# arielnetworks/tidal-wave

Hardware: AMD Instinct MI355X
Metric: image-pairs/sec @1080p Farneback (default params), 1/2/4/8 MI355X (higher is better)
Workload: dtype f32

## Files before the change

include/twflow_debug.h:

```cpp
#ifndef TWFLOW_DEBUG_H
#define TWFLOW_DEBUG_H

#include "twflow.h"

#ifdef __cplusplus
extern "C" {
#endif

int tw_debug_graphs(tw_engine* e);

tw_status tw_debug_check_size(int width, int height);

int tw_debug_occupancy(char* buf, int cap);

int tw_debug_stamps(tw_engine* e, unsigned long long* out);

int tw_debug_stamps_ex(tw_engine* e, unsigned long long* out, int n);

tw_status tw_debug_copy_rate(tw_engine* e, size_t bytes, int reps, double* gbps);

enum tw_debug_family {
    TW_DF_PYR_K3 = 0,
    TW_DF_PYR_K3F,
    TW_DF_PYR_23,
// ... 17 lines not shown
    TW_DF_SPAN_SCAN,
    TW_DF_PNG_UNFILTER,
    TW_DF_SPAN_SCAN_SEG,
    TW_DF_BLUR_SOLVE4Q,
    TW_DF_PAIR_SAME,
    TW_DF_RESIZE_U8,
    TW_DF_FLOW_INIT,
    TW_DF_FLOW_EXPORT,
    TW_DF_COUNT
};

int tw_debug_launch_counts(tw_engine* e, unsigned long long* counts, unsigned long long* last_z, int n, int reset);

int tw_debug_flow_iter_plan(const tw_engine* e, int width, int height, int npairs, int* out, int n);

int tw_debug_blur_plan(const tw_engine* e, int width, int height, int level, int npairs, int update, int quads, int* out, int n);

int tw_debug_same_flags(tw_engine* e, unsigned* out, int n);

tw_status tw_debug_png_kernel_time(tw_engine* e, const tw_png_rows* img, int waves, int iters, float* avg_us);

const char* tw_debug_family_name(int family);

int tw_debug_memory(tw_engine* e, unsigned long long* out, int n);

#ifdef __cplusplus
}
#endif
#endif
```

tidal-wave_amd/csrc/twflow.hip:

```cpp
#include "twflow_kernels.hip.h"

#include <hip/hip_runtime.h>
#include <unistd.h>

#include <dlfcn.h>
#include <float.h>
#include <math.h>
#include <stdio.h>
#include <stdlib.h>
#include <string.h>

#include <array>
#include <chrono>
#include <map>
#include <mutex>
#include <string>
#include <tuple>
#include <utility>
#include <vector>

#include "../../include/twflow.h"
#include "../../include/twflow_debug.h"

using namespace twk;
// ... 77 lines not shown
            if (sx >= sw - 1) { fx = 0; sx = sw - 1; }
        }
        t.xofs[dx] = sx;
        t.alpha[2 * dx] = 1.f - fx;
        t.alpha[2 * dx + 1] = fx;
    }
    for (int dy = 0; dy < dh; dy++) {
        float fy = (float)((dy + 0.5) * scale_y - 0.5);
        int sy = cv_floor(fy);
        fy -= sy;
        t.yofs[dy] = sy;
        t.beta[2 * dy] = 1.f - fy;
        t.beta[2 * dy + 1] = fy;
    }
}

struct AreaTab {
    int mode = 2, ix = 1, iy = 1;
    std::vector<int> xstart, xsi, ystart, ysi;
    std::vector<float> xalpha, ybeta;
};
void area_tab_1d(int ssize, int dsize, double scale, std::vector<int>& start, std::vector<int>& si, std::vector<float>& alpha)
{
    start.assign(dsize + 1, 0);
    si.clear();
    alpha.clear();
    for (int dx = 0; dx < dsize; dx++) {
        start[dx] = (int)si.size();
        const double fsx1 = dx * scale;
        const double fsx2 = fsx1 + scale;
// ... 127 lines not shown
    int w = 0, h = 0, ld = 0;
    long long ps = 0;
    double sigma = 0, scale = 1;
    int ksize = 3;
    int chunk = 1;
    int *d_xofs = nullptr, *d_yofs = nullptr;
    float *d_alpha = nullptr, *d_beta = nullptr, *d_kern = nullptr;
    int mode = 1, xmax = 0, nrows_max = 0;
    float h_kern[3] = {0, 0, 0};
    std::vector<float> h_taps;
    int pitch_b = 0;
    int gen_th = PYR_TH, gen_nrows_max = 0;
    int *d_uxofs = nullptr, *d_uyofs = nullptr;
    float *d_ualpha = nullptr, *d_ubeta = nullptr;
    int uxmax = 0;
};

struct Plan {
    int w0 = 0, h0 = 0;
    bool fused23 = false;
    float k19[24] = {0}, k9[16] = {0};
    int levels = 0;
    std::vector<LevelPlan> lv;
    int init_mode = 0, init_ix = 1, init_iy = 1, init_tw = 0;
    int *d_ixs = nullptr, *d_ixi = nullptr, *d_iys = nullptr, *d_iyi = nullptr;
    float *d_ixa = nullptr, *d_iyb = nullptr;
    std::vector<void*> owned;
    size_t owned_bytes = 0;
    unsigned long long last_use = 0;
};
// ... 504 lines not shown
            (s = upload_vec(e, pl, t.alpha, &L.d_alpha)) || (s = upload_vec(e, pl, t.beta, &L.d_beta)) ||
            (s = upload_vec(e, pl, kern, &L.d_kern))) {
            free_plan(pl);
            return s;
        }
        if (k < pl->levels) {
            const LevelPlan& P = pl->lv[k + 1];
            ResizeTab u;
            make_resize_tab(P.w, P.h, L.w, L.h, u);
            if (u.mode == 2) {
                e->err = "unexpected area-fast flow resize";
                free_plan(pl);
                return TW_E_UNSUPPORTED;
            }
            L.uxmax = u.xmax;
            if ((s = upload_vec(e, pl, u.xofs, &L.d_uxofs)) || (s = upload_vec(e, pl, u.yofs, &L.d_uyofs)) ||
                (s = upload_vec(e, pl, u.alpha, &L.d_ualpha)) || (s = upload_vec(e, pl, u.beta, &L.d_ubeta))) {
                free_plan(pl);
                return s;
            }
        }
    }
    {
        const LevelPlan& C = pl->lv[pl->levels];
        AreaTab t;
        make_area_tab(w0, h0, C.w, C.h, t);
        pl->init_mode = t.mode;
        pl->init_ix = t.ix;
        pl->init_iy = t.iy;
        if (t.mode == 1) {
// ... 406 lines not shown
    return e->p.pyrIterations > 0 && e->scan_fused && span == 10 && e->win_m == 15 && !e->box;
}
int balanced_launch_pairs(int n, int chunk)
{
    const int nlaunch = (n + chunk - 1) / chunk;
    return nlaunch > 0 ? (n + nlaunch - 1) / nlaunch : 1;
}
struct FlowUps {
    const float* prev;
    int pw, ph, pld;
    long long pfps;
    const int *xofs, *yofs;
    const float *alpha, *beta;
    int xmax;
    float scale;
};
template <typename A>
void set_upsample(A& a, const FlowUps& u)
{
    a.prev = u.prev;
    a.pw = u.pw;
    a.ph = u.ph;
    a.pld = u.pld;
    a.pfps = u.pfps;
    a.xofs = u.xofs;
    a.alpha = u.alpha;
    a.yofs = u.yofs;
    a.beta = u.beta;
    a.xmax = u.xmax;
    a.scale = u.scale;
// ... 28 lines not shown
        if (sg > 1 && nt < e->fi_minsteps) break;
        const long long wgs = (long long)nstrips * sg * npairs;
        const long long rounds = (wgs + slots - 1) / slots;
        const double cost = (double)rounds * (nt + 7 * 0.25);
        if (cost < best_cost) {
            best_cost = cost;
            best_seg = sg;
        }
    }
    FlowIterPlan fp;
    fp.strips = nstrips;
    fp.nt = (nsteps + best_seg - 1) / best_seg;
    fp.segments = (nsteps + fp.nt - 1) / fp.nt;
    fp.nt_last = nsteps - (fp.segments - 1) * fp.nt;
    return fp;
}
void launch_flow_iter(tw_engine* e, hipStream_t st, int w, int h, int ld, long long ps, const float* R, const float* flow_in,
                      long long fps_in, float* flow_out, long long fps_out, const FlowUps* ups, int npairs, int level,
                      const unsigned* same = nullptr)
{
    FlowIterArgs a;
    memset(&a, 0, sizeof(a));
    a.same = same;
    a.R = R;
    a.flow_in = flow_in;
    a.flow_out = flow_out;
    a.w = w;
    a.h = h;
    a.ld = ld;
    a.ps = ps;
// ... 6 lines not shown
    a.dbg = (unsigned long long*)e->dbg_stamps;
#endif
    const FlowIterPlan fp = flow_iter_plan(e, w, h, npairs);
    a.nt = fp.nt;
    const dim3 grid(fp.strips, fp.segments, npairs);
    ProfScope pscope(e, st, TW_K_BLUR_SOLVE, level);
    if (ups) set_upsample(a, *ups);
#ifdef TW_VARIANTS
    if (e->fi_nt == 512) {
        if (ups) TW_LAUNCH(e, TW_DF_FLOW_ITER_UPS, (tw_flow_iter<15, 1, 512>), grid, dim3(512), 0, st, a);
        else if (a.zero_flow) TW_LAUNCH(e, TW_DF_FLOW_ITER_ZERO, (tw_flow_iter<15, 2, 512>), grid, dim3(512), 0, st, a);
        else TW_LAUNCH(e, TW_DF_FLOW_ITER, (tw_flow_iter<15, 0, 512>), grid, dim3(512), 0, st, a);
        return;
    }
#endif
    if (ups) {
        TW_LAUNCH(e, TW_DF_FLOW_ITER_UPS, (tw_flow_iter<15, 1>), grid, dim3(1024), 0, st, a);
    } else if (a.zero_flow) {
        TW_LAUNCH(e, TW_DF_FLOW_ITER_ZERO, (tw_flow_iter<15, 2>), grid, dim3(1024), 0, st, a);
    } else {
        TW_LAUNCH(e, TW_DF_FLOW_ITER, (tw_flow_iter<15, 0>), grid, dim3(1024), 0, st, a);
    }
}

#ifndef TW_4Y_ILP
#define TW_4Y_ILP 2, 2, 2
#endif
struct BlurKernel {
    void (*kern)(BlurArgs);
    int family;
    int block;
// ... 175 lines not shown
    } else {
        void (*const kern)(BlurArgs) = c.k->kern;
        TW_LAUNCH(e, c.k->family, kern, c.grid, dim3(c.k->block), c.lds, st, a);
    }
}

void launch_update(tw_engine* e, hipStream_t st, const Plan* pl, int k, const float* R, float* flow,
                   const float* prev, float* M, int npairs, const SideJob* side = nullptr, bool* side_used = nullptr,
                   bool init_flow = false)
{
    const LevelPlan& L = pl->lv[k];
    const bool up = k < pl->levels;
    FlowUps ups;
    if (up) {
        const LevelPlan& P = pl->lv[k + 1];
        ups = FlowUps{prev, P.w, P.h, P.ld, P.ps, L.d_uxofs, L.d_uyofs, L.d_ualpha, L.d_ubeta, L.uxmax, (float)(1. / e->p.pyrScale)};
    }
    UpdArgs a = upd_args(R, flow, M, L.w, L.h, L.ld, L.ps, up ? &ups : nullptr);
    a.store_flow = e->p.pyrIterations == 0 ? 1 : 0;
    ProfScope pscope(e, st, TW_K_UPDATE_MATRICES, k);
    if (up) {
        launch_upd_kernel<true>(e, st, L.w, L.h, npairs, a, side, side_used);
    } else {
        a.zero_flow = init_flow ? 0 : 1;
        launch_upd_kernel<false>(e, st, L.w, L.h, npairs, a, side, side_used);
    }
}

void launch_area_init(tw_engine* e, hipStream_t st, const Plan* pl, float* flow, int j0, int nc)
{
    const LevelPlan& L = pl->lv[pl->levels];
// ... 695 lines not shown
        side_next++;
    }


    void enqueue_flow_iter_chain(const LevelChunk& ch)
    {
        const int k = ch.k, nc = ch.nc;
        const LevelPlan& L = pl->lv[k];
        const int nfi = ch.grid_only ? it - 1 : it;
        float* buf[2] = {ch.flow_cur, ch.M0};
        if (ch.init_lv) launch_area_init(e, ch.ls, pl, buf[nfi & 1], ch.j0, nc);
        FlowUps ups;
        if (k < pl->levels) {
            const LevelPlan& Pv = pl->lv[k + 1];
            ups = FlowUps{ch.flow_prev, Pv.w, Pv.h, Pv.ld, Pv.ps, L.d_uxofs, L.d_uyofs, L.d_ualpha, L.d_ubeta, L.uxmax,
                          (float)(1. / e->p.pyrScale)};
        }
        for (int i = 0; i < nfi; i++) {
            float* out = buf[(nfi - 1 - i) & 1];
            const float* in = i == 0 ? (ch.init_lv ? buf[nfi & 1] : nullptr) : buf[(nfi - i) & 1];
            launch_flow_iter(e, ch.ls, L.w, L.h, L.ld, L.ps, ch.R, in, L.ps, out, L.ps,
                             (i == 0 && k < pl->levels) ? &ups : nullptr, nc, k, same_flags_of(ch));
        }
        if (!ch.grid_only) return;
        UpdArgs u;
        memset(&u, 0, sizeof(u));
        u.R = ch.R;
        u.flow = ch.flow_cur;
        u.M = ch.M1;
        u.w = L.w;
        u.h = L.h;
// ... 1473 lines not shown
    const char* why = "";
    return size_status(width, height, &why);
}

extern "C" int tw_debug_flow_iter_plan(const tw_engine* e, int width, int height, int npairs, int* out, int n)
{
    if (!e) return -1;
    if (!out || width < 1 || height < 1 || npairs < 1) return 0;
    const FlowIterPlan fp = flow_iter_plan(e, width, height, npairs);
    const int v[4] = {fp.strips, fp.segments, fp.nt, fp.nt_last};
    int i = 0;
    for (; i < n && i < 4; i++) out[i] = v[i];
    return i;
}

extern "C" int tw_debug_blur_plan(const tw_engine* e, int width, int height, int level, int npairs, int update, int quads, int* out, int n)
{
    if (!e) return -1;
    if (!out || width < 1 || height < 1 || npairs < 1) return 0;
    const BlurChoice c = choose_blur(e, width, height, npairs, level, update != 0, quads != 0);
    const int v[9] = {c.k->family, c.k->block, c.k->tw, c.k->th, c.xsh, (int)c.grid.x, (int)c.grid.y, c.small, c.forced ? 1 : 0};
    int i = 0;
    for (; i < n && i < 9; i++) out[i] = v[i];
    return i;
}

extern "C" int tw_debug_launch_counts(tw_engine* e, unsigned long long* counts, unsigned long long* last_z, int n, int reset)
{
    if (!e) return -1;
    for (int i = 0; i < n && i < TW_DF_COUNT; i++) {
// ... 218 lines not shown
        switch (kclass) {
            case TW_K_PYR:
                e->img_aligned4 = (npx0 % 4 == 0) ? 1 : 0;
                launch_pyr(e, st, pl, level, tab, width, I, 2 * npairs);
                break;
            case TW_K_POLYEXP: return launch_polyexp(e, st, L.w, L.h, L.ld, L.ps, I, R, 2 * npairs, level);
            case TW_K_UPDATE_MATRICES: launch_update(e, st, pl, level, R, fl, pf, M0, npairs); break;
            case TW_K_BLUR_SOLVE:
                if (flags & 12) {
                    if (!flow_iter_eligible(e, L.w, L.h)) return TW_E_UNSUPPORTED;
                    FlowUps ups;
                    const bool up = (flags & 8) && level < pl->levels;
                    if (up) {
                        const LevelPlan& Pv = pl->lv[level + 1];
                        ups = FlowUps{pf, Pv.w, Pv.h, Pv.ld, Pv.ps, L.d_uxofs, L.d_uyofs, L.d_ualpha, L.d_ubeta, L.uxmax,
                                      (float)(1. / e->p.pyrScale)};
                    }
                    launch_flow_iter(e, st, L.w, L.h, L.ld, L.ps, R, up ? nullptr : fl, L.ps, M1, L.ps, up ? &ups : nullptr,
                                     npairs, level);
                    break;
                }
                launch_blur(e, st, BlurLaunch{L.w, L.h, L.ld, L.ps, (i & 1) ? M1 : M0, (i & 1) ? M0 : M1, fl, R, (flags & 2) ? 0 : 1,
                                              level, npairs});
                break;
            case TW_K_SCAN: {
                GatherArgs g;
                g.flow = fl; g.fzs = 2 * L.ps; g.fps = L.ps; g.ld = L.ld; g.span = span;
                g.gw = (L.w + span - 1) / span; g.gh = (L.h + span - 1) / span; g.g = grid;
                TW_LAUNCH(e, TW_DF_SPAN_GATHER, tw_span_gather, dim3((g.gw + 63) / 64, (g.gh + 3) / 4, npairs), dim3(256), 0, st, g);
                ScanArgs a;
                a.g = grid; a.span = span; a.gw = g.gw; a.gh = g.gh; a.thr2 = 4.0; a.count = cnt;
// ... 51 lines not shown
{
    ResizeTab u;
    make_resize_tab(pw, ph, w, h, u);
    if (u.mode == 2) return TW_E_UNSUPPORTED;
    const int pld = round_up(pw, 32);
    const long long pps = (long long)pld * ph;
    float* d_p = t.alloc<float>(pps * 2);
    int *d_xo = t.alloc<int>(w), *d_yo = t.alloc<int>(h);
    float *d_al = t.alloc<float>(2 * (size_t)w), *d_be = t.alloc<float>(2 * (size_t)h);
    if (!d_p || !d_xo || !d_yo || !d_al || !d_be) return TW_E_NOMEM;
    TW_TRY(up_planes(e, d_p, pld, pps, prev2, pw, ph, 2));
    TW_TRY(h2d_sync(e, d_xo, u.xofs.data(), (size_t)w * 4));
    TW_TRY(h2d_sync(e, d_yo, u.yofs.data(), (size_t)h * 4));
    TW_TRY(h2d_sync(e, d_al, u.alpha.data(), (size_t)w * 8));
    TW_TRY(h2d_sync(e, d_be, u.beta.data(), (size_t)h * 8));
    *ups = FlowUps{d_p, pw, ph, pld, pps, d_xo, d_yo, d_al, d_be, u.xmax, (float)(1. / e->p.pyrScale)};
    return TW_OK;
}
}

extern "C" {

tw_status tw_stage_pyr_level(tw_engine* e, const uint8_t* img, int w0, int h0, int level, float* I, int* w, int* h)
{
    if (!e || !img || !I) return TW_E_BAD_PARAMETER;
    tw_status r = check_dims(e, w0, h0);
    if (r) return r;
    TW_HIP(e, hipSetDevice(e->device));
    Plan* pl = nullptr;
    if ((r = get_plan(e, w0, h0, &pl))) return r;
    if (level < 0 || level > pl->levels) return TW_E_BAD_PARAMETER;
// ... 319 lines not shown
```

tidal-wave_amd/csrc/twflow_kernels.hip.h:

```cpp
#pragma once
#include <hip/hip_runtime.h>
#include <stdint.h>
#include <type_traits>

namespace twk {

typedef float __attribute__((ext_vector_type(4))) f32x4;
typedef const float __attribute__((address_space(1))) * gptr_cf;
typedef const char __attribute__((address_space(1))) * gptr_cc;

__device__ __forceinline__ gptr_cf sgpr_base(const float* p)
{
    gptr_cf g = (gptr_cf)p;
    asm volatile("" : "+s"(g));
    return g;
}
__device__ __forceinline__ float gload(gptr_cf row, unsigned byte_off)
{
    return *(gptr_cf)((gptr_cc)row + byte_off);
}
typedef float __attribute__((address_space(1))) * gptr_f;
typedef char __attribute__((address_space(1))) * gptr_c;
__device__ __forceinline__ gptr_f sgpr_base_w(float* p)
{
// ... 1859 lines not shown
                    }
                }
            }
        }
    }
}
template <int MH, int COLS, int HALO, int TH, bool FUSED, int VILP = 2, int HILP = 2, int SUNROLL = 2, bool QPRE = true, bool VPRE = true>
__global__ __launch_bounds__(COLS) __attribute__((amdgpu_waves_per_eu(4, 8))) void tw_blur_solve4(BlurArgs a)
{
    __shared__ __attribute__((aligned(16))) float sm[5][TH][COLS];
    tw_blur_solve4_body<MH, COLS, HALO, TH, FUSED, VILP, HILP, SUNROLL, QPRE, VPRE>(a, hw_grid(), hw_block(), sm);
}

constexpr int FI_TH = 5, FI_SC = 190, FI_PITCH = 192;
constexpr int FI_SC_512 = 94, FI_PITCH_512 = 96;
struct FlowIterArgs {
    const float* R;
    const float* flow_in;
    float* flow_out;
    int w, h, ld;
    long long ps, fps_in, fps_out;
    int nt;
    int zero_flow;
    const float* prev;
    int pw, ph, pld;
    long long pfps;
    const int* xofs;
    const float* alpha;
    const int* yofs;
    const float* beta;
// ... 9 lines not shown
#define TW_FI_SKIP(bit) (a.dbg_skip & (bit))
#define TW_FI_SYNC() do { if (!TW_FI_SKIP(16)) __syncthreads(); } while (0)
#define TW_FI_STAMP(i)                                                                                                   \
    do {                                                                                                                 \
        if (a.dbg && (tid == 0 || tid == NT / 2 + 64) && fi_blin < 32 && st >= 40 && st < 48)                              \
            a.dbg[(((size_t)fi_blin * 2 + (tid ? 1 : 0)) * 8 + (st - 40)) * 8 + (i)] = __builtin_amdgcn_s_memtime();       \
    } while (0)
#else
#define TW_FI_SKIP(bit) false
#define TW_FI_SYNC() __syncthreads()
#define TW_FI_STAMP(i) do { } while (0)
#endif
template <int MH, int MODE, int NT = 1024>
__global__ __launch_bounds__(NT) __attribute__((amdgpu_waves_per_eu(4, 4))) void tw_flow_iter(FlowIterArgs a)
{
    constexpr bool UPS = MODE == 1;
#ifndef TW_FI_DEEP
#define TW_FI_DEEP 1
#endif
    constexpr bool DEEP = TW_FI_DEEP && MODE != 1 && NT == 1024;
#ifndef TW_FI_DIST
#define TW_FI_DIST 0
#endif
#define TW_FI_P(ph, sl) ((ph) * 8 + (sl))
    constexpr int DIST[4][10] = {
        {TW_FI_P(0, 0), TW_FI_P(0, 0), TW_FI_P(1, 0), TW_FI_P(1, 0), TW_FI_P(1, 1), TW_FI_P(1, 1), TW_FI_P(2, 0), TW_FI_P(2, 0), TW_FI_P(2, 0), TW_FI_P(2, 0)},
        {TW_FI_P(0, 1), TW_FI_P(0, 3), TW_FI_P(1, 0), TW_FI_P(1, 1), TW_FI_P(1, 2), TW_FI_P(1, 3), TW_FI_P(2, 0), TW_FI_P(2, 0), TW_FI_P(2, 1), TW_FI_P(2, 1)},
        {TW_FI_P(2, 0), TW_FI_P(2, 0), TW_FI_P(2, 0), TW_FI_P(2, 0), TW_FI_P(2, 0), TW_FI_P(2, 0), TW_FI_P(2, 0), TW_FI_P(2, 0), TW_FI_P(2, 0), TW_FI_P(2, 0)},
        {TW_FI_P(0, 0), TW_FI_P(0, 0), TW_FI_P(0, 1), TW_FI_P(0, 1), TW_FI_P(0, 2), TW_FI_P(0, 2), TW_FI_P(0, 3), TW_FI_P(0, 3), TW_FI_P(0, 4), TW_FI_P(0, 4)},
    };
#ifndef TW_FI_UDIST
#define TW_FI_UDIST 1
#endif
    constexpr int UDIST[2][15] = {
        {TW_FI_P(0, 0), TW_FI_P(0, 0), TW_FI_P(0, 1), TW_FI_P(0, 1), TW_FI_P(0, 2), TW_FI_P(0, 2), TW_FI_P(1, 0), TW_FI_P(1, 0), TW_FI_P(1, 1), TW_FI_P(1, 1),
         TW_FI_P(0, 0), TW_FI_P(0, 1), TW_FI_P(0, 2), TW_FI_P(0, 3), TW_FI_P(0, 4)},
        {TW_FI_P(0, 0), TW_FI_P(0, 0), TW_FI_P(0, 1), TW_FI_P(0, 2), TW_FI_P(0, 3), TW_FI_P(0, 4), TW_FI_P(1, 0), TW_FI_P(1, 1), TW_FI_P(1, 2), TW_FI_P(1, 3),
         TW_FI_P(2, 1), TW_FI_P(2, 1), TW_FI_P(2, 1), TW_FI_P(2, 1), TW_FI_P(2, 1)},
    };
    constexpr int TH = FI_TH, SC = NT == 1024 ? FI_SC : FI_SC_512, P = NT == 1024 ? FI_PITCH : FI_PITCH_512, OUT = SC - 2 * MH,
                  RING = TH + 2 * MH, NCH = RING / TH, NB = NCH + 1;
    static_assert(RING % TH == 0 && SC <= P && TH * SC <= NT && TH == 5 && OUT % 4 == 0 && 5 * TH * (OUT / 4) <= NT && (NB & (NB - 1)) == 0, "geometry");
    constexpr int VWAVES = (TH * SC + 63) / 64;
    constexpr bool SPLIT = VWAVES * 64 < NT;
    __shared__ __attribute__((aligned(16))) float blk[NB][5][TH][P];
    const int tid = threadIdx.x;
    int bx, seg, z;
    xcd_remap(bx, seg, z);
    const unsigned fi_blin = blockIdx.x + gridDim.x * (blockIdx.y + gridDim.y * blockIdx.z);
    (void)fi_blin;
    const WinCoef& c = a.c;
    const float* __restrict__ R0 = a.R + (long long)(2 * z) * 5 * a.ps;
    const float* __restrict__ R1 = R0 + ((a.same && a.same[z]) ? 0 : 5 * a.ps);
    const float* __restrict__ fin = a.flow_in + (long long)z * 2 * a.fps_in;
    float* __restrict__ fout = a.flow_out + (long long)z * 2 * a.fps_out;
    const bool cth = tid < TH * SC;
    const int cr = cth ? tid / SC : 0, cc = cth ? tid - cr * SC : 0;
    const int xc = clampi(bx * OUT - MH + cc, 0, a.w - 1);
    const int ys = seg * a.nt * TH;
    const int nsteps = min(a.nt, (a.h - ys + TH - 1) / TH);
// ... 42 lines not shown
            f.p[1] = bload(rsp, b0 + sx1b, 0u);
            f.p[2] = bload(rsp, b1 + sxb, 0u);
            f.p[3] = bload(rsp, b1 + sx1b, 0u);
            f.p[4] = bload(rsp, b0 + sxb, prev_p1);
            f.p[5] = bload(rsp, b0 + sx1b, prev_p1);
            f.p[6] = bload(rsp, b1 + sxb, prev_p1);
            f.p[7] = bload(rsp, b1 + sx1b, prev_p1);
        } else if constexpr (MODE == 2) {
            f.p[0] = f.p[1] = 0.f;
        } else {
            const unsigned o = (unsigned)(yc * a.ld + xc) * 4u;
            f.p[0] = bload(rsf, o, 0u);
            f.p[1] = bload(rsf, o, fin_p1);
        }
    };
    auto flow_value = [&](const FlowIn& f, float& dx, float& dy) {
        if constexpr (UPS) {
            const float t0x = two ? f.p[0] * ua0 + f.p[1] * ua1 : f.p[0] * 1.f;
            const float t1x = two ? f.p[2] * ua0 + f.p[3] * ua1 : f.p[2] * 1.f;
            const float t0y = two ? f.p[4] * ua0 + f.p[5] * ua1 : f.p[4] * 1.f;
            const float t1y = two ? f.p[6] * ua0 + f.p[7] * ua1 : f.p[6] * 1.f;
            dx = (t0x * f.b0 + t1x * f.b1) * a.scale + 0.f;
            dy = (t0y * f.b0 + t1y * f.b1) * a.scale + 0.f;
        } else {
            asm volatile("v_mov_b32 %0, %2\n\tv_mov_b32 %1, %3" : "=&v"(dx), "=&v"(dy) : "v"(f.p[0]), "v"(f.p[1]));
        }
    };
    gptr_cf r0b[5], r1b[5];
#pragma unroll
    for (int ch = 0; ch < 5; ch++) {
        r0b[ch] = sgpr_base(R0 + ch * a.ps);
        r1b[ch] = sgpr_base(R1 + ch * a.ps);
    }
    unsigned go0 = 0, go1 = 0;
    unsigned gq = 0;
    auto gather_r0 = [&](int ch, float q[5]) { q[ch] = gload(r0b[ch], gq); };
    auto gather_head = [&](int k, float dx, float dy, float q[5], UpdTaps& T, bool with_r0) {
        const int yc = row_of(k);
        gq = (unsigned)(yc * a.ld + xc) * 4u;
        if (with_r0) {
// ... 50 lines not shown
        ytab_issue(0);
        flow_issue(0, fcur);
        ytab_issue(1);
#pragma unroll 1
        for (int k = 0; k < NCH; k++) {
            flow_issue(k + 1, fnext);
            ytab_issue(k + 2);
            flow_value(fcur, dx, dy);
            gather_issue(k, dx, dy, q, T);
            combine_store(k, dx, dy, q, T);
            fcur = fnext;
        }
        if constexpr (DEEP) {
            FlowIn f2;
            flow_issue(NCH + 1, f2);
            ytab_issue(NCH + 2);
            flow_value(fnext, dx, dy);
            gather_head(NCH, dx, dy, q, T, false);
#pragma unroll
            for (int ch = 0; ch < 5; ch++) gather_plane(ch, T);
            flow_value(f2, dxb, dyb);
            gather_head(NCH + 1, dxb, dyb, q, Tb, false);
        } else {
        flow_value(fnext, dx, dy);
        gather_head(NCH, dx, dy, q, T, true);
        }
    }
    __syncthreads();

    constexpr int NQ = OUT / 4;
    const bool hth = tid < 5 * TH * NQ;
// ... 57 lines not shown
                    for (int u = 0; u < 15; u++)
                        if (UDIST[TW_FI_UDIST][u] == TW_FI_P(1, j)) {
                            if (u < 10) gather_half(u >> 1, u & 1, Tl);
                            else gather_r0(u - 10, ql);
                        }
                } else {
                    if (j < 2) gather_plane(HPLANE0 + j, Tl);
                }
            }
            __builtin_amdgcn_sched_barrier(0);
        }
        *(f32x4*)&blk[s0][hp][hr][4 * hq] = o;
    };

    if (SPLIT && tid >= VWAVES * 64) {
#pragma unroll 1
        for (int st = 0; st < nsteps; st++) {
            const int s0 = st & (NB - 1), bX = (st + NCH) & (NB - 1);
            TW_FI_SYNC();
            if (hth && !TW_FI_SKIP(4)) h_phase(s0, bX, std::false_type(), T, q);
            TW_FI_SYNC();
            s_phase(st, s0);
            TW_FI_SYNC();
        }
        return;
    }

    auto step = [&](int st, float (&qc)[5], float (&qn)[5]) {
        const bool more = st + 1 < nsteps;
        const int s0 = st & (NB - 1), bX = (st + NCH) & (NB - 1);
        TW_FI_STAMP(0);
        if (cth) {
            flow_issue(st + NCH + 1, fnext);
            ytab_issue(st + NCH + 2);
            gq = (unsigned)(row_of(st + NCH + 1) * a.ld + xc) * 4u;
            __builtin_amdgcn_sched_barrier(0);
            float wv[RING];
#pragma unroll
            for (int j = 0; j < NCH; j++) {
                const float* bj = &blk[(s0 + j) & (NB - 1)][cr][0][cc];
#pragma unroll
                for (int r = 0; r < TH; r++) wv[TH * j + r] = bj[r * P];
            }
            float* vout = &blk[bX][cr][0][cc];
#pragma unroll
            for (int r = 0; r < TH; r++) {
                float sv = wv[r + MH] * c.k[0];
#pragma unroll
                for (int i = 1; i <= MH; i++) sv += (wv[r + MH + i] + wv[r + MH - i]) * c.k[i];
// ... 23 lines not shown
        TW_FI_STAMP(4);

        s_phase(st, s0);
        __builtin_amdgcn_sched_barrier(0);
        TW_FI_STAMP(5);
        if (cth) {
            if (more && !TW_FI_SKIP(1)) combine_store(st + NCH, dx, dy, qc, T);
            __builtin_amdgcn_sched_barrier(0);
            if constexpr (UPS) {
#pragma unroll
                for (int u = 10; u < 15; u++)
                    if (UDIST[TW_FI_UDIST][u] == TW_FI_P(2, 1)) gather_r0(u - 10, qn);
                __builtin_amdgcn_sched_barrier(0);
            }
            TW_FI_STAMP(6);
            flow_value(fnext, dx, dy);
            gather_head(st + NCH + 1, dx, dy, qn, T, false);
            __builtin_amdgcn_sched_barrier(0);
        }
        TW_FI_STAMP(7);
        TW_FI_SYNC();
    };
    auto step_deep = [&](int st, float& dxc, float& dyc, UpdTaps& Tc, float& dxn, float& dyn, UpdTaps& Tn) {
        const bool more = st + 1 < nsteps;
        const int s0 = st & (NB - 1), bX = (st + NCH) & (NB - 1);
        TW_FI_STAMP(0);
        if (cth) {
            flow_issue(st + NCH + 2, fnext);
            ytab_issue(st + NCH + 3);
            gq = (unsigned)(row_of(st + NCH) * a.ld + xc) * 4u;
            __builtin_amdgcn_sched_barrier(0);
            float wv[RING];
#pragma unroll
            for (int j = 0; j < NCH; j++) {
                const float* bj = &blk[(s0 + j) & (NB - 1)][cr][0][cc];
#pragma unroll
                for (int r = 0; r < TH; r++) wv[TH * j + r] = bj[r * P];
            }
            float* vout = &blk[bX][cr][0][cc];
#pragma unroll
            for (int r = 0; r < TH; r++) {
                float sv = wv[r + MH] * c.k[0];
#pragma unroll
                for (int i = 1; i <= MH; i++) sv += (wv[r + MH + i] + wv[r + MH - i]) * c.k[i];
// ... 16 lines not shown
        s_phase(st, s0);
        __builtin_amdgcn_sched_barrier(0);
        TW_FI_STAMP(5);
        if (cth) {
#pragma unroll
            for (int u = 0; u < 10; u++)
                if (DIST[TW_FI_DIST][u] == TW_FI_P(2, 0)) gather_half(u >> 1, u & 1, Tn);
            __builtin_amdgcn_sched_barrier(0);
            if (more && !TW_FI_SKIP(1)) combine_store(st + NCH, dxc, dyc, q, Tc);
            __builtin_amdgcn_sched_barrier(0);
#pragma unroll
            for (int u = 0; u < 10; u++)
                if (DIST[TW_FI_DIST][u] == TW_FI_P(2, 1)) gather_half(u >> 1, u & 1, Tn);
            __builtin_amdgcn_sched_barrier(0);
            TW_FI_STAMP(6);
            flow_value(fnext, dxc, dyc);
            gather_head(st + NCH + 2, dxc, dyc, q, Tc, false);
            __builtin_amdgcn_sched_barrier(0);
        }
        TW_FI_STAMP(7);
        TW_FI_SYNC();
    };
    if constexpr (DEEP) {
        int st = 0;
#pragma unroll 1
        for (; st + 1 < nsteps; st += 2) {
            step_deep(st, dx, dy, T, dxb, dyb, Tb);
            step_deep(st + 1, dxb, dyb, Tb, dx, dy, T);
        }
        if (st < nsteps) step_deep(st, dx, dy, T, dxb, dyb, Tb);
        return;
// ... 1913 lines not shown
```

tidal-wave_amd/twflow.py:

```python
import collections
import ctypes as C
import os

import numpy as np

_HERE = os.path.dirname(os.path.abspath(__file__))
LIB_PATH = os.path.join(_HERE, "libtwflow.so")

TW_OK, TW_E_BAD_PARAMETER, TW_E_BAD_IMAGE_FORMAT, TW_E_DONT_MATCH_SIZE = 0, 1, 2, 3
TW_E_DEVICE, TW_E_NOMEM, TW_E_UNSUPPORTED, TW_E_BUSY = 4, 5, 6, 7
K_PYR, K_POLYEXP, K_UPDATE_MATRICES, K_BLUR_SOLVE, K_SCAN = 0, 1, 2, 3, 4
KERNEL_NAMES = {K_PYR: "tw_pyr_level", K_POLYEXP: "tw_polyexp", K_UPDATE_MATRICES: "tw_update_matrices",
                K_BLUR_SOLVE: "tw_blur_solve", K_SCAN: "tw_span_scan"}


class Params(C.Structure):
    _fields_ = [("pyrScale", C.c_double), ("pyrLevels", C.c_int), ("winSize", C.c_int),
                ("pyrIterations", C.c_int), ("polyN", C.c_int), ("polySigma", C.c_double),
                ("flags", C.c_int)]


class Vector(C.Structure):
    _fields_ = [("x", C.c_int), ("y", C.c_int), ("dx", C.c_double), ("dy", C.c_double)]

# ... 21 lines not shown
OPT_POLYEXP_F32 = 2

SYMBOLS = [
    "tw_default_params", "tw_abi_version", "tw_has_variants", "tw_device_count", "tw_device_pci_bus_id", "tw_engine_create", "tw_engine_destroy", "tw_strerror",
    "tw_last_error", "tw_flow_u8", "tw_diff_u8", "tw_submit_u8", "tw_submit_png8", "tw_submit_dev", "tw_flush", "tw_wait",
    "tw_submit_u8_flow", "tw_submit_png8_flow", "tw_submit_dev_flow",
    "tw_submit_u8_flow_init", "tw_submit_png8_flow_init", "tw_submit_dev_flow_init",
    "tw_submit_u8_sized", "tw_submit_png8_sized", "tw_submit_dev_sized", "tw_stage_resize_u8",
    "tw_png_on_device", "tw_submit_png", "tw_stage_png_decode",
    "tw_grid_capacity", "tw_dev_alloc", "tw_dev_free", "tw_dev_upload", "tw_dev_download", "tw_host_alloc", "tw_host_free", "tw_host_register", "tw_host_unregister", "tw_set_option",
    "tw_prof_select", "tw_prof_read",
    "tw_algorithmic_bytes", "tw_algorithmic_bytes_launch", "tw_level_runs_flow_iter", "tw_algorithmic_bytes_pair", "tw_min_traffic_bytes_pair", "tw_num_levels", "tw_level_chunk", "tw_bench_stage", "tw_stage_pyr_level", "tw_stage_pyr_fused23", "tw_stage_pyr_fused01",
    "tw_stage_png_unfilter", "tw_stage_polyexp", "tw_stage_update_matrices", "tw_stage_flow_upsample_update", "tw_stage_blur_solve", "tw_stage_flow_iter",
    "tw_debug_graphs", "tw_debug_occupancy", "tw_debug_stamps", "tw_debug_stamps_ex", "tw_debug_copy_rate",
    "tw_debug_launch_counts", "tw_debug_family_name", "tw_debug_memory", "tw_debug_check_size", "tw_debug_flow_iter_plan",
    "tw_debug_blur_plan", "tw_debug_same_flags", "tw_debug_png_kernel_time",
]


PNG_PLAIN_GRAY = -1


class PngRows(C.Structure):
    _fields_ = [("rows", C.POINTER(C.c_uint8)), ("width", C.c_int), ("height", C.c_int), ("color_type", C.c_int),
                ("bit_depth", C.c_int), ("palette", C.POINTER(C.c_uint8)), ("palette_entries", C.c_int)]

    def __init__(self, rows, width, height, color_type=PNG_PLAIN_GRAY, bit_depth=8, palette=None, palette_entries=None):
        super().__init__()
        self._rows = np.ascontiguousarray(rows, np.uint8)
        self._palette = None if palette is None else np.ascontiguousarray(palette, np.uint8)
# ... 128 lines not shown
    L.tw_algorithmic_bytes_launch.argtypes = [vp, C.c_int, C.c_int, C.c_int, C.c_int, C.c_int]
    L.tw_algorithmic_bytes_launch.restype = C.c_double
    L.tw_level_runs_flow_iter.argtypes = [vp, C.c_int, C.c_int, C.c_int, C.c_int]
    L.tw_level_runs_flow_iter.restype = C.c_int
    u64p = C.POINTER(C.c_uint64)
    L.tw_debug_launch_counts.argtypes = [vp, u64p, u64p, C.c_int, C.c_int]
    L.tw_debug_launch_counts.restype = C.c_int
    L.tw_debug_family_name.argtypes = [C.c_int]
    L.tw_debug_family_name.restype = C.c_char_p
    L.tw_debug_memory.argtypes = [vp, u64p, C.c_int]
    L.tw_debug_memory.restype = C.c_int
    L.tw_debug_check_size.argtypes = [C.c_int, C.c_int]
    L.tw_debug_check_size.restype = C.c_int
    L.tw_debug_flow_iter_plan.argtypes = [vp, C.c_int, C.c_int, C.c_int, ip, C.c_int]
    L.tw_debug_flow_iter_plan.restype = C.c_int
    L.tw_debug_blur_plan.argtypes = [vp, C.c_int, C.c_int, C.c_int, C.c_int, C.c_int, C.c_int, ip, C.c_int]
    L.tw_debug_blur_plan.restype = C.c_int
    L.tw_debug_same_flags.argtypes = [vp, C.POINTER(C.c_uint), C.c_int]
    L.tw_debug_same_flags.restype = C.c_int
    return L


FlowIterPlan = collections.namedtuple("FlowIterPlan", "strips segments nt nt_last")
BlurPlan = collections.namedtuple("BlurPlan", "family block tile_cols rows xsh grid_x grid_y small forced")


class LaunchCounts(dict):

    def flow_iter(self):
        return self["tw_flow_iter"] + self["tw_flow_iter_ups"] + self["tw_flow_iter_zero"]


def abi_version():
    return lib().tw_abi_version()


def default_params(**kw):
    p = Params()
# ... 363 lines not shown
    def algorithmic_bytes(self, kclass, level, w, h, npairs=None):
        if npairs is None:
            return self._L.tw_algorithmic_bytes(self._h, kclass, level, w, h)
        return self._L.tw_algorithmic_bytes_launch(self._h, kclass, level, w, h, npairs)

    def level_runs_flow_iter(self, w, h, level, npairs):
        return self._L.tw_level_runs_flow_iter(self._h, w, h, level, npairs) == 1

    def flow_iter_plan(self, w, h, npairs=1):
        v = (C.c_int * 4)()
        n = self._L.tw_debug_flow_iter_plan(self._h, w, h, npairs, v, 4)
        if n != 4:
            raise TwError(TW_E_BAD_PARAMETER, "tw_debug_flow_iter_plan(%d, %d, %d) returned %d" % (w, h, npairs, n))
        return FlowIterPlan(*v)

    def blur_plan(self, w, h, level=-1, npairs=1, update=False, quads=False):
        v = (C.c_int * 9)()
        n = self._L.tw_debug_blur_plan(self._h, w, h, level, npairs, int(bool(update)), int(bool(quads)), v, 9)
        if n != 9:
            raise TwError(TW_E_BAD_PARAMETER, "tw_debug_blur_plan(%d, %d, %d, %d) returned %d" % (w, h, level, npairs, n))
        return BlurPlan(self._L.tw_debug_family_name(v[0]).decode(), *v[1:8], bool(v[8]))

    def same_flags(self):
        v = (C.c_uint * self.slots)()
        n = self._L.tw_debug_same_flags(self._h, v, self.slots)
        if n < 0:
            raise TwError(TW_E_DEVICE, "tw_debug_same_flags returned %d" % n)
        return [int(v[i]) for i in range(n)]

    def launch_counts(self, reset=False):
# ... 100 lines not shown
```

Baseline: 4983.

## Stage upsampled previous-level flow in LDS via idle wave in flow_iter

Adds a staged variant of the upsampling flow-iteration kernel in which the spare wave beyond the compute waves prefetches the previous-level flow rows and row interpolation weights into a shared-memory staging array one step ahead. Compute threads then read the bilinear taps from LDS instead of issuing per-thread global gathers and y-table loads on the critical path. The plan decides per level whether the source column span fits the staging width, and otherwise falls back to the old path. This costs extra LDS and adds a producer pipeline that could affect occupancy or synchronization.

Measured after the change: 5007 (median of 6 runs). No clear change (+0.5%).

```diff
diff --git a/include/twflow_debug.h b/include/twflow_debug.h
--- a/include/twflow_debug.h
+++ b/include/twflow_debug.h
@@ -55,6 +55,8 @@
 
 int tw_debug_flow_iter_plan(const tw_engine* e, int width, int height, int npairs, int* out, int n);
 
+int tw_debug_flow_iter_ups_plan(const tw_engine* e, int prev_width, int prev_height, int width, int height, int* out, int n);
+
 int tw_debug_blur_plan(const tw_engine* e, int width, int height, int level, int npairs, int update, int quads, int* out, int n);
 
 int tw_debug_same_flags(tw_engine* e, unsigned* out, int n);
diff --git a/tidal-wave_amd/csrc/twflow.hip b/tidal-wave_amd/csrc/twflow.hip
--- a/tidal-wave_amd/csrc/twflow.hip
+++ b/tidal-wave_amd/csrc/twflow.hip
@@ -115,6 +115,12 @@
         t.beta[2 * dy + 1] = fy;
     }
 }
+
+struct FlowIterStage {
+    int rows, cols, bytes;
+    bool staged;
+};
+FlowIterStage flow_iter_ups_stage(const std::vector<int>& xofs, int w);
 
 struct AreaTab {
     int mode = 2, ix = 1, iy = 1;
@@ -272,6 +278,7 @@
     int *d_uxofs = nullptr, *d_uyofs = nullptr;
     float *d_ualpha = nullptr, *d_ubeta = nullptr;
     int uxmax = 0;
+    bool ustaged = false;
 };
 
 struct Plan {
@@ -806,6 +813,7 @@
                 return TW_E_UNSUPPORTED;
             }
             L.uxmax = u.xmax;
+            L.ustaged = flow_iter_ups_stage(u.xofs, L.w).staged;
             if ((s = upload_vec(e, pl, u.xofs, &L.d_uxofs)) || (s = upload_vec(e, pl, u.yofs, &L.d_uyofs)) ||
                 (s = upload_vec(e, pl, u.alpha, &L.d_ualpha)) || (s = upload_vec(e, pl, u.beta, &L.d_ubeta))) {
                 free_plan(pl);
@@ -1242,6 +1250,7 @@
     const float *alpha, *beta;
     int xmax;
     float scale;
+    bool staged;
 };
 template <typename A>
 void set_upsample(A& a, const FlowUps& u)
@@ -1300,6 +1309,21 @@
     fp.segments = (nsteps + fp.nt - 1) / fp.nt;
     fp.nt_last = nsteps - (fp.segments - 1) * fp.nt;
     return fp;
+}
+FlowIterStage flow_iter_ups_stage(const std::vector<int>& xofs, int w)
+{
+    const int OUT = FI_SC - 30;
+    int cols = 0;
+    for (int bx = 0; bx * OUT < w; bx++) {
+        const int xl = std::min(std::max(bx * OUT - 15, 0), w - 1), xr = std::min(bx * OUT - 15 + FI_SC - 1, w - 1);
+        cols = std::max(cols, xofs[xr] - xofs[xl] + 2);
+    }
+    FlowIterStage s;
+    s.rows = 2 * FI_TH;
+    s.cols = cols;
+    s.bytes = (2 * s.rows * cols + 2 * FI_TH + 2 * FI_PITCH) * 4;
+    s.staged = cols <= FI_STG_COLS;
+    return s;
 }
 void launch_flow_iter(tw_engine* e, hipStream_t st, int w, int h, int ld, long long ps, const float* R, const float* flow_in,
                       long long fps_in, float* flow_out, long long fps_out, const FlowUps* ups, int npairs, int level,
@@ -1336,7 +1360,9 @@
         return;
     }
 #endif
-    if (ups) {
+    if (ups && ups->staged) {
+        TW_LAUNCH(e, TW_DF_FLOW_ITER_UPS, (tw_flow_iter<15, 3>), grid, dim3(1024), 0, st, a);
+    } else if (ups) {
         TW_LAUNCH(e, TW_DF_FLOW_ITER_UPS, (tw_flow_iter<15, 1>), grid, dim3(1024), 0, st, a);
     } else if (a.zero_flow) {
         TW_LAUNCH(e, TW_DF_FLOW_ITER_ZERO, (tw_flow_iter<15, 2>), grid, dim3(1024), 0, st, a);
@@ -1542,7 +1568,7 @@
     FlowUps ups;
     if (up) {
         const LevelPlan& P = pl->lv[k + 1];
-        ups = FlowUps{prev, P.w, P.h, P.ld, P.ps, L.d_uxofs, L.d_uyofs, L.d_ualpha, L.d_ubeta, L.uxmax, (float)(1. / e->p.pyrScale)};
+        ups = FlowUps{prev, P.w, P.h, P.ld, P.ps, L.d_uxofs, L.d_uyofs, L.d_ualpha, L.d_ubeta, L.uxmax, (float)(1. / e->p.pyrScale), L.ustaged};
     }
     UpdArgs a = upd_args(R, flow, M, L.w, L.h, L.ld, L.ps, up ? &ups : nullptr);
     a.store_flow = e->p.pyrIterations == 0 ? 1 : 0;
@@ -2268,7 +2294,7 @@
         if (k < pl->levels) {
             const LevelPlan& Pv = pl->lv[k + 1];
             ups = FlowUps{ch.flow_prev, Pv.w, Pv.h, Pv.ld, Pv.ps, L.d_uxofs, L.d_uyofs, L.d_ualpha, L.d_ubeta, L.uxmax,
-                          (float)(1. / e->p.pyrScale)};
+                          (float)(1. / e->p.pyrScale), L.ustaged};
         }
         for (int i = 0; i < nfi; i++) {
             float* out = buf[(nfi - 1 - i) & 1];
@@ -3772,6 +3798,20 @@
     return i;
 }
 
+extern "C" int tw_debug_flow_iter_ups_plan(const tw_engine* e, int prev_width, int prev_height, int width, int height, int* out, int n)
+{
+    if (!e) return -1;
+    if (!out || prev_width < 1 || prev_height < 1 || width < 1 || height < 1) return 0;
+    ResizeTab u;
+    make_resize_tab(prev_width, prev_height, width, height, u);
+    if (u.mode == 2) return 0;
+    const FlowIterStage s = flow_iter_ups_stage(u.xofs, width);
+    const int v[5] = {s.staged && e->fi_nt != 512 ? 1 : 0, s.rows, s.cols, s.bytes, FI_STG_DWORDS * 4};
+    int i = 0;
+    for (; i < n && i < 5; i++) out[i] = v[i];
+    return i;
+}
+
 extern "C" int tw_debug_blur_plan(const tw_engine* e, int width, int height, int level, int npairs, int update, int quads, int* out, int n)
 {
     if (!e) return -1;
@@ -4020,7 +4060,7 @@
                     if (up) {
                         const LevelPlan& Pv = pl->lv[level + 1];
                         ups = FlowUps{pf, Pv.w, Pv.h, Pv.ld, Pv.ps, L.d_uxofs, L.d_uyofs, L.d_ualpha, L.d_ubeta, L.uxmax,
-                                      (float)(1. / e->p.pyrScale)};
+                                      (float)(1. / e->p.pyrScale), L.ustaged};
                     }
                     launch_flow_iter(e, st, L.w, L.h, L.ld, L.ps, R, up ? nullptr : fl, L.ps, M1, L.ps, up ? &ups : nullptr,
                                      npairs, level);
@@ -4102,7 +4142,7 @@
     TW_TRY(h2d_sync(e, d_yo, u.yofs.data(), (size_t)h * 4));
     TW_TRY(h2d_sync(e, d_al, u.alpha.data(), (size_t)w * 8));
     TW_TRY(h2d_sync(e, d_be, u.beta.data(), (size_t)h * 8));
-    *ups = FlowUps{d_p, pw, ph, pld, pps, d_xo, d_yo, d_al, d_be, u.xmax, (float)(1. / e->p.pyrScale)};
+    *ups = FlowUps{d_p, pw, ph, pld, pps, d_xo, d_yo, d_al, d_be, u.xmax, (float)(1. / e->p.pyrScale), flow_iter_ups_stage(u.xofs, w).staged};
     return TW_OK;
 }
 }
diff --git a/tidal-wave_amd/csrc/twflow_kernels.hip.h b/tidal-wave_amd/csrc/twflow_kernels.hip.h
--- a/tidal-wave_amd/csrc/twflow_kernels.hip.h
+++ b/tidal-wave_amd/csrc/twflow_kernels.hip.h
@@ -1897,6 +1897,10 @@
 
 constexpr int FI_TH = 5, FI_SC = 190, FI_PITCH = 192;
 constexpr int FI_SC_512 = 94, FI_PITCH_512 = 96;
+constexpr int FI_STG_COLS = 98, FI_STG_LINES = 4 * FI_TH;
+constexpr int FI_STG_ROWTAB = FI_STG_LINES * FI_STG_COLS, FI_STG_COLTAB = FI_STG_ROWTAB + 2 * FI_TH;
+constexpr int FI_STG_DWORDS = FI_STG_COLTAB + 2 * FI_PITCH;
+constexpr int FI_LDS_BYTES = 163840;
 struct FlowIterArgs {
     const float* R;
     const float* flow_in;
@@ -1936,11 +1940,16 @@
 template <int MH, int MODE, int NT = 1024>
 __global__ __launch_bounds__(NT) __attribute__((amdgpu_waves_per_eu(4, 4))) void tw_flow_iter(FlowIterArgs a)
 {
-    constexpr bool UPS = MODE == 1;
+    constexpr bool STG = MODE == 3;
+    constexpr bool UPS = MODE == 1 || STG;
+    static_assert(!STG || NT == 1024, "the staged upsample needs wave 15");
 #ifndef TW_FI_DEEP
 #define TW_FI_DEEP 1
 #endif
-    constexpr bool DEEP = TW_FI_DEEP && MODE != 1 && NT == 1024;
+#ifndef TW_FI_STG_DEEP
+#define TW_FI_STG_DEEP 1
+#endif
+    constexpr bool DEEP = TW_FI_DEEP && MODE != 1 && (!STG || TW_FI_STG_DEEP) && NT == 1024;
 #ifndef TW_FI_DIST
 #define TW_FI_DIST 0
 #endif
@@ -1966,6 +1975,10 @@
     constexpr int VWAVES = (TH * SC + 63) / 64;
     constexpr bool SPLIT = VWAVES * 64 < NT;
     __shared__ __attribute__((aligned(16))) float blk[NB][5][TH][P];
+    __shared__ __attribute__((aligned(16))) float stg[STG ? FI_STG_DWORDS : 1];
+    static_assert(!STG || sizeof(blk) + FI_STG_DWORDS * 4 <= FI_LDS_BYTES, "staging array");
+    constexpr int CP = FI_STG_COLS;
+    constexpr int KOFF = NCH + (DEEP ? 2 : 1);
     const int tid = threadIdx.x;
     int bx, seg, z;
     xcd_remap(bx, seg, z);
@@ -2038,7 +2051,7 @@
             f.p[1] = bload(rsf, o, fin_p1);
         }
     };
-    auto flow_value = [&](const FlowIn& f, float& dx, float& dy) {
+    auto ups_value = [&](const FlowIn& f, bool two, float ua0, float ua1, float& dx, float& dy) {
         if constexpr (UPS) {
             const float t0x = two ? f.p[0] * ua0 + f.p[1] * ua1 : f.p[0] * 1.f;
             const float t1x = two ? f.p[2] * ua0 + f.p[3] * ua1 : f.p[2] * 1.f;
@@ -2046,8 +2059,80 @@
             const float t1y = two ? f.p[6] * ua0 + f.p[7] * ua1 : f.p[6] * 1.f;
             dx = (t0x * f.b0 + t1x * f.b1) * a.scale + 0.f;
             dy = (t0y * f.b0 + t1y * f.b1) * a.scale + 0.f;
+        }
+    };
+    auto flow_value = [&](const FlowIn& f, float& dx, float& dy) {
+        if constexpr (UPS) {
+            ups_value(f, two, ua0, ua1, dx, dy);
         } else {
             asm volatile("v_mov_b32 %0, %2\n\tv_mov_b32 %1, %3" : "=&v"(dx), "=&v"(dy) : "v"(f.p[0]), "v"(f.p[1]));
+        }
+    };
+    const int xlo = STG ? clampi(bx * OUT - MH, 0, a.w - 1) : 0;
+    int sxbase = 0;
+    unsigned stg_tap = 0;
+    if constexpr (STG) {
+        sxbase = a.xofs[xlo];
+        stg_tap = (unsigned)(2 * cr * CP + sx - sxbase) | (two ? 0u : 0x80000000u);
+        if (tid < SC) {
+            float* ct = &stg[FI_STG_COLTAB + xc - xlo];
+            ct[0] = ua0;
+            ct[P] = ua1;
+        }
+    }
+    auto flow_staged = [&](float& dx, float& dy) {
+        if constexpr (STG) {
+            const float* ct = &stg[FI_STG_COLTAB + xc - xlo];
+            const float* sp = &stg[stg_tap & 0x7FFFFFFFu];
+            FlowIn f;
+#pragma unroll
+            for (int pl = 0; pl < 2; pl++) {
+                f.p[4 * pl] = sp[pl * 2 * TH * CP];
+                f.p[4 * pl + 1] = sp[pl * 2 * TH * CP + 1];
+                f.p[4 * pl + 2] = sp[pl * 2 * TH * CP + CP];
+                f.p[4 * pl + 3] = sp[pl * 2 * TH * CP + CP + 1];
+            }
+            f.b0 = stg[FI_STG_ROWTAB + 2 * cr];
+            f.b1 = stg[FI_STG_ROWTAB + 2 * cr + 1];
+            ups_value(f, !(stg_tap >> 31), ct[0], ct[P], dx, dy);
+        }
+    };
+    const int wl = tid & 63;
+    const unsigned svo0 = STG ? (unsigned)min(sxbase + wl, a.pw - 1) * 4u : 0u, svo1 = STG ? (unsigned)min(sxbase + wl + 64, a.pw - 1) * 4u : 0u;
+    float sreg[STG ? 2 * FI_STG_LINES : 1];
+    float sb0 = 0.f, sb1 = 0.f;
+    int ssy = 0;
+    auto stg_row = [&](int k) { return clampi(ys - MH + TH * k + min(wl, TH - 1), 0, a.h - 1); };
+    auto stg_ytab = [&](int k) { ssy = a.yofs[stg_row(k)]; };
+    auto stg_issue = [&](int k) {
+        const int yc = stg_row(k);
+        sb0 = a.beta[2 * yc];
+        sb1 = a.beta[2 * yc + 1];
+#pragma unroll
+        for (int r = 0; r < TH; r++) {
+            const int sy = __builtin_amdgcn_readlane(ssy, r);
+#pragma unroll
+            for (int hf = 0; hf < 2; hf++) {
+                const unsigned so = (unsigned)(clampi(sy + hf, 0, a.ph - 1) * a.pld) * 4u;
+#pragma unroll
+                for (int pl = 0; pl < 2; pl++) {
+                    const int line = pl * 2 * TH + 2 * r + hf;
+                    sreg[2 * line] = bload(rsp, svo0, so + (pl ? prev_p1 : 0u));
+                    sreg[2 * line + 1] = bload(rsp, svo1, so + (pl ? prev_p1 : 0u));
+                }
+            }
+        }
+    };
+    auto stg_write = [&]() {
+#pragma unroll
+        for (int line = 0; line < FI_STG_LINES; line++) stg[line * CP + wl] = sreg[2 * line];
+        if (wl + 64 < CP) {
+#pragma unroll
+            for (int line = 0; line < FI_STG_LINES; line++) stg[line * CP + wl + 64] = sreg[2 * line + 1];
+        }
+        if (wl < TH) {
+            stg[FI_STG_ROWTAB + 2 * wl] = sb0;
+            stg[FI_STG_ROWTAB + 2 * wl + 1] = sb1;
         }
     };
     gptr_cf r0b[5], r1b[5];
@@ -2128,7 +2213,7 @@
         if constexpr (DEEP) {
             FlowIn f2;
             flow_issue(NCH + 1, f2);
-            ytab_issue(NCH + 2);
+            if constexpr (!STG) ytab_issue(NCH + 2);
             flow_value(fnext, dx, dy);
             gather_head(NCH, dx, dy, q, T, false);
 #pragma unroll
@@ -2216,9 +2301,19 @@
     };
 
     if (SPLIT && tid >= VWAVES * 64) {
+        if constexpr (STG) {
+            stg_ytab(KOFF);
+            stg_issue(KOFF);
+            stg_ytab(KOFF + 1);
+        }
 #pragma unroll 1
         for (int st = 0; st < nsteps; st++) {
             const int s0 = st & (NB - 1), bX = (st + NCH) & (NB - 1);
+            if constexpr (STG) {
+                stg_write();
+                stg_issue(st + KOFF + 1);
+                stg_ytab(st + KOFF + 2);
+            }
             TW_FI_SYNC();
             if (hth && !TW_FI_SKIP(4)) h_phase(s0, bX, std::false_type(), T, q);
             TW_FI_SYNC();
@@ -2233,8 +2328,10 @@
         const int s0 = st & (NB - 1), bX = (st + NCH) & (NB - 1);
         TW_FI_STAMP(0);
         if (cth) {
-            flow_issue(st + NCH + 1, fnext);
-            ytab_issue(st + NCH + 2);
+            if constexpr (!STG) {
+                flow_issue(st + NCH + 1, fnext);
+                ytab_issue(st + NCH + 2);
+            }
             gq = (unsigned)(row_of(st + NCH + 1) * a.ld + xc) * 4u;
             __builtin_amdgcn_sched_barrier(0);
             float wv[RING];
@@ -2288,7 +2385,8 @@
                 __builtin_amdgcn_sched_barrier(0);
             }
             TW_FI_STAMP(6);
-            flow_value(fnext, dx, dy);
+            if constexpr (STG) flow_staged(dx, dy);
+            else flow_value(fnext, dx, dy);
             gather_head(st + NCH + 1, dx, dy, qn, T, false);
             __builtin_amdgcn_sched_barrier(0);
         }
@@ -2300,8 +2398,10 @@
         const int s0 = st & (NB - 1), bX = (st + NCH) & (NB - 1);
         TW_FI_STAMP(0);
         if (cth) {
-            flow_issue(st + NCH + 2, fnext);
-            ytab_issue(st + NCH + 3);
+            if constexpr (!STG) {
+                flow_issue(st + NCH + 2, fnext);
+                ytab_issue(st + NCH + 3);
+            }
             gq = (unsigned)(row_of(st + NCH) * a.ld + xc) * 4u;
             __builtin_amdgcn_sched_barrier(0);
             float wv[RING];
@@ -2348,7 +2448,8 @@
                 if (DIST[TW_FI_DIST][u] == TW_FI_P(2, 1)) gather_half(u >> 1, u & 1, Tn);
             __builtin_amdgcn_sched_barrier(0);
             TW_FI_STAMP(6);
-            flow_value(fnext, dxc, dyc);
+            if constexpr (STG) flow_staged(dxc, dyc);
+            else flow_value(fnext, dxc, dyc);
             gather_head(st + NCH + 2, dxc, dyc, q, Tc, false);
             __builtin_amdgcn_sched_barrier(0);
         }
diff --git a/tidal-wave_amd/twflow.py b/tidal-wave_amd/twflow.py
--- a/tidal-wave_amd/twflow.py
+++ b/tidal-wave_amd/twflow.py
@@ -59,6 +59,7 @@
     "tw_stage_png_unfilter", "tw_stage_polyexp", "tw_stage_update_matrices", "tw_stage_flow_upsample_update", "tw_stage_blur_solve", "tw_stage_flow_iter",
     "tw_debug_graphs", "tw_debug_occupancy", "tw_debug_stamps", "tw_debug_stamps_ex", "tw_debug_copy_rate",
     "tw_debug_launch_counts", "tw_debug_family_name", "tw_debug_memory", "tw_debug_check_size", "tw_debug_flow_iter_plan",
+    "tw_debug_flow_iter_ups_plan",
     "tw_debug_blur_plan", "tw_debug_same_flags", "tw_debug_png_kernel_time",
 ]
 
@@ -217,6 +218,8 @@
     L.tw_debug_check_size.restype = C.c_int
     L.tw_debug_flow_iter_plan.argtypes = [vp, C.c_int, C.c_int, C.c_int, ip, C.c_int]
     L.tw_debug_flow_iter_plan.restype = C.c_int
+    L.tw_debug_flow_iter_ups_plan.argtypes = [vp, C.c_int, C.c_int, C.c_int, C.c_int, ip, C.c_int]
+    L.tw_debug_flow_iter_ups_plan.restype = C.c_int
     L.tw_debug_blur_plan.argtypes = [vp, C.c_int, C.c_int, C.c_int, C.c_int, C.c_int, C.c_int, ip, C.c_int]
     L.tw_debug_blur_plan.restype = C.c_int
     L.tw_debug_same_flags.argtypes = [vp, C.POINTER(C.c_uint), C.c_int]
@@ -225,6 +228,7 @@
 
 
 FlowIterPlan = collections.namedtuple("FlowIterPlan", "strips segments nt nt_last")
+FlowIterUpsPlan = collections.namedtuple("FlowIterUpsPlan", "staged rows cols bytes capacity")
 BlurPlan = collections.namedtuple("BlurPlan", "family block tile_cols rows xsh grid_x grid_y small forced")
 
 
@@ -618,6 +622,13 @@
             raise TwError(TW_E_BAD_PARAMETER, "tw_debug_flow_iter_plan(%d, %d, %d) returned %d" % (w, h, npairs, n))
         return FlowIterPlan(*v)
 
+    def flow_iter_ups_plan(self, pw, ph, w, h):
+        v = (C.c_int * 5)()
+        n = self._L.tw_debug_flow_iter_ups_plan(self._h, pw, ph, w, h, v, 5)
+        if n != 5:
+            raise TwError(TW_E_BAD_PARAMETER, "tw_debug_flow_iter_ups_plan(%d, %d, %d, %d) returned %d" % (pw, ph, w, h, n))
+        return FlowIterUpsPlan(bool(v[0]), *v[1:])
+
     def blur_plan(self, w, h, level=-1, npairs=1, update=False, quads=False):
         v = (C.c_int * 9)()
         n = self._L.tw_debug_blur_plan(self._h, w, h, level, npairs, int(bool(update)), int(bool(quads)), v, 9)
```
